# TobiasDeBruijn/UU-INFOGR-Raytracer

Hardware: AMD Instinct MI355X
Metric: Mray/s (primary+shadow+reflect) and fps at 1920×1080, 1/2/4/8 MI355X (higher is better)
Workload: dtype f32

## Files before the change

uu-infogr-raytracer_amd/csrc/rt_api.cpp:

```cpp
#include <hip/hip_runtime.h>

#include <algorithm>
#include <climits>
#include <cmath>
#include <cstdarg>
#include <cstdio>
#include <cstdlib>
#include <cstring>
#include <dlfcn.h>
#include <link.h>
#include <new>
#include <string>
#include <vector>

#include "../../include/raytracer_hip.h"
#include "rt_bands.h"
#include "rt_internal.h"
#include "rt_progressive.h"
#include "rt_scene.h"
#include "rt_view.h"

using namespace rtk;

namespace {
// ... 314 lines not shown

int view_params(rt_ctx* ctx, int W, int H, LaunchParams& lp, int ss = 0) {
    const int VH = ctx->view_height > 0 ? ctx->view_height << ss : H;
    if (H > VH)
        return fail(ctx, RT_ERR_INVALID_ARG, "frame height %d above the view height %d", H >> ss, ctx->view_height);
    if (ctx->view_ok && ctx->view_w == W && ctx->view_h == VH && ctx->view_rows == H &&
        std::memcmp(&ctx->view_cam, &ctx->cam, sizeof ctx->cam) == 0) {
        copy_view(ctx->view_lp, lp);
        return RT_OK;
    }
    int rc = view_fill(ctx, ctx->cam, W, VH, lp);
    if (rc != RT_OK) return rc;
    lp.row_order_n = row_order(lp, ctx->layout, lp.row_order);
    lp.H = H;
    copy_view(lp, ctx->view_lp);
    ctx->view_cam = ctx->cam, ctx->view_w = W, ctx->view_h = VH, ctx->view_rows = H, ctx->view_ok = true;
    return RT_OK;
}

void scene_params(const rt_ctx* ctx, const Device& d, LaunchParams& lp) {
    const SceneLayout& L = ctx->layout;
    const char* base = (const char*)d.d_scene;
    lp.sph = (const DevSphere*)(base + L.off_sph);
    lp.mat = (const DevMaterial*)(base + L.off_mat);
    lp.pl = (const DevPlane*)(base + L.off_pl);
    lp.li = (const DevLight*)(base + L.off_li);
    lp.scull = (const DevSphereCull*)(base + L.off_cull);
    lp.shcull = L.has_shcull ? (const DevShadowCull*)(base + L.off_shcull) : nullptr;
    lp.shg = L.has_shg ? (const DevShadowGrid*)(base + L.off_shg) : nullptr;
    lp.shgrid = L.has_shg ? (const unsigned long long*)(base + L.off_shgrid) : nullptr;
    lp.shslab = L.has_shg ? (const unsigned long long*)(base + L.off_shslab) : nullptr;
    lp.clus = L.n_clus ? (const DevCluster*)(base + L.off_clus) : nullptr;
    lp.shpre = L.has_shpre ? (const DevShadowCull*)(base + L.off_shpre) : nullptr;
    lp.n_clus = L.n_clus;
    lp.S = L.S, lp.P = L.P, lp.L = L.L, lp.limit = L.limit;
    lp.lights_a2_ok = L.lights_a2_ok ? 1 : 0;
    lp.uniform_plane = L.uniform_plane ? 1 : 0;
    lp.counters = ctx->counting ? d.d_counters : nullptr;
}

int view_tables(rt_ctx* ctx, Device& d, LaunchParams& lp, int ss = 0) {
    const int VH = ctx->view_height > 0 ? ctx->view_height << ss : lp.H;
    if (d.tab_w != lp.W || d.tab_h != VH || d.tab_pw != lp.pw || d.tab_ph != lp.ph || !d.d_view_tab) {
        std::vector<float> t((size_t)lp.W + (size_t)VH);
        view_table_values(lp.W, VH, lp.pw, lp.ph, t.data());
        HIP_TRY(ctx, hipDeviceSynchronize());
        int rc = grow(ctx, (void**)&d.d_view_tab, &d.view_tab_cap, t.size() * sizeof(float));
        if (rc != RT_OK) return rc;
        HIP_TRY(ctx, hipMemcpy(d.d_view_tab, t.data(), t.size() * sizeof(float), hipMemcpyHostToDevice));
        d.tab_w = lp.W, d.tab_h = VH, d.tab_pw = lp.pw, d.tab_ph = lp.ph;
    }
    lp.lxt = d.d_view_tab;
    lp.lyt = d.d_view_tab + lp.W;
    return RT_OK;
}

constexpr int ORDER_CANDIDATES = 4, ORDER_SAMPLES = 7;
constexpr float ORDER_MARGIN = 1.01f;
constexpr uint64_t ORDER_RETUNE = 1u << 14;

void order_collect(Device& d) {
    Device::OrderTuner& t = d.order;
    size_t keep = 0;
    for (size_t i = 0; i < t.pending.size(); ++i) {
        Device::OrderTuner::Probe& pr = t.pending[i];
        if (hipEventQuery(pr.b) != hipSuccess) {
// ... 538 lines not shown
        if (d.d_counters_diag) (void)hipFree(d.d_counters_diag);
        if (d.d_view_tab) (void)hipFree(d.d_view_tab);
        if (d.d_prog) (void)hipFree(d.d_prog);
        if (d.order.tiles.d_order) (void)hipFree(d.order.tiles.d_order);
        if (d.order.tiles.d_cost) (void)hipFree(d.order.tiles.d_cost);
        if (d.d_stage) (void)hipFree(d.d_stage);
        if (d.async_stream) (void)hipStreamDestroy(d.async_stream);
        if (d.stream) (void)hipStreamDestroy(d.stream);
    }
    delete ctx;
}

int rt_set_scene(rt_ctx* ctx, const rt_sphere* spheres, int n_spheres, const rt_plane* planes, int n_planes,
                 const rt_light* lights, int n_lights, rt_vec3 ambient, int recursion_limit) {
    if (!ctx) return fail(nullptr, RT_ERR_INVALID_ARG, "NULL context");
    if (n_spheres < 0 || n_planes < 0 || n_lights < 0 || (n_spheres && !spheres) || (n_planes && !planes) ||
        (n_lights && !lights))
        return fail(ctx, RT_ERR_INVALID_ARG, "rt_set_scene: bad primitive arrays");
    if (recursion_limit < 0) return fail(ctx, RT_ERR_INVALID_ARG, "recursion_limit must be >= 0");
    if (n_lights > RT_MAX_LIGHTS)
        return fail(ctx, RT_ERR_UNSUPPORTED, "n_lights %d > RT_MAX_LIGHTS (%d)", n_lights, RT_MAX_LIGHTS);
    if (recursion_limit > RT_MAX_RECURSION_LIMIT)
        return fail(ctx, RT_ERR_UNSUPPORTED, "recursion_limit %d > RT_MAX_RECURSION_LIMIT (%d)", recursion_limit,
                    RT_MAX_RECURSION_LIMIT);

    auto off = [](const char* name) {
        const char* v = std::getenv(name);
        return v && std::strcmp(v, "0") == 0;
    };
    SceneOptions opt;
    opt.shadow_grid = !off("RT_SHADOW_GRID");
    if (const char* cv = std::getenv("RT_TRACE_CLUSTERS")) opt.cluster_size = std::atoi(cv);
    opt.shadow_pre = !off("RT_SHADOW_PRE");
    opt.mirror_box = !off("RT_MIRROR_BOX");
    opt.dark_skip = !off("RT_DARK_SKIP");
    opt.prim_foot = !off("RT_PRIM_FOOT");
    opt.uniform_plane = !off("RT_UNIFORM_PLANE");
    SceneLayout L = scene_build(spheres, n_spheres, planes, n_planes, lights, n_lights, ambient, recursion_limit, opt);
    for (Device& d : ctx->dev) {
        DeviceGuard guard(d.id);
        HIP_TRY(ctx, hipDeviceSynchronize());
        int rc = grow(ctx, &d.d_scene, &d.scene_cap, L.bytes);
        if (rc != RT_OK) return rc;
        HIP_TRY(ctx, hipMemcpy(d.d_scene, L.host_blob.data(), L.bytes, hipMemcpyHostToDevice));
    }
    ctx->layout = std::move(L);
    ctx->has_scene = true;
    ctx->view_ok = false;
    ctx->scene_gen++;
    return RT_OK;
}

int rt_set_view_height(rt_ctx* ctx, int view_height) {
    if (!ctx || view_height < 0) return fail(ctx, RT_ERR_INVALID_ARG, "rt_set_view_height: bad arguments");
    ctx->view_height = view_height;
    return RT_OK;
}

int rt_set_supersampling(rt_ctx* ctx, int k) {
    if (!ctx) return fail(nullptr, RT_ERR_INVALID_ARG, "rt_set_supersampling: NULL context");
    if (k != 1 && k != 2 && k != 4 && k != 8)
        return fail(ctx, RT_ERR_INVALID_ARG, "rt_set_supersampling: factor %d is not 1, 2, 4 or 8", k);
    ctx->ss_log2 = k == 8 ? 3 : k == 4 ? 2 : k == 2 ? 1 : 0;
    return RT_OK;
}

// ... 991 lines not shown
```

uu-infogr-raytracer_amd/csrc/rt_internal.h:

```cpp
#pragma once
#include <stdint.h>

#include "rt_resolve.h"

namespace rtk {

struct DevSphere {
    float cx, cy, cz, r2;
};

enum : uint32_t { MAT_MIRROR = 1u, MAT_DIFFUSE = 2u, MAT_SPEC = 4u, MAT_DARK_OK = 8u };

enum : uint32_t { POW_GENERIC = 0u, POW_ONE = 1u, POW_HALF = 2u, POW_TWO = 3u };

struct DevMaterial {
    float kd[3];
    float amb[3];
    float ks[3];
    float n;
    float km[3];
    uint32_t flags;
    uint32_t pow_kind;
    uint32_t pad;
};
// ... 2 lines not shown
    float cx, cy, cz, cn;
    float nx, ny, nz, pad0;
    float e1x, e1y, e1z, pad1;
    float e2x, e2y, e2z, pad2;
};

struct DevLight {
    float px, py, pz, intensity;
    float a;
    float a2;
    float a4;
    float sh_t;
    float ax, ay, az, pad1;
    float ux, uy, uz, pad2;
    float vx, vy, vz, pad3;
};

struct DevSphereCull {
    float cx, cy, cz, rr;
};

struct DevCluster {
    float cx, cy, cz, R;
    unsigned long long members;
    unsigned long long pad;
};
constexpr int CLUSTER_SIZE = 8;
constexpr int MAX_CLUSTERS = 32;

struct DevShadowCull {
    float cu, cv, ca, rr;
};
constexpr long long SHADOW_CULL_MAX_ENTRIES = 1LL << 16;

constexpr int SHADOW_MERGE_L = 4;
constexpr int SHGRID_N = 64;
constexpr int SHGRID_SLABS = 32;
struct DevShadowGrid {
    float su, ou, sv, ov;
    float sa, oa;
    float bound;
    float far_k;
    float far_b;
    float bu0, bu1, bv0, bv1;
    float pad;
    unsigned long long always;
};

constexpr int COUNTER_SLOTS = 256;
constexpr int COUNTER_STRIDE = 8;
constexpr int COUNTER_WORDS = COUNTER_SLOTS * COUNTER_STRIDE;
enum : int { CNT_REFLECT = 1, CNT_SHADOW = 2, CNT_SHADOW_RUN = 3, CNT_SPHERE_RUN = 4, CNT_PLANE_RUN = 5 };
enum : int { CNT_EXTRA_PRIMARY = 0 };

struct PrimBox {
    int x0, x1, y0, y1;
};

struct PrimConst {
    float ocx, ocy, ocz, c;
};
constexpr int MAX_PRIM_CONST = 64;
struct PlaneFoot {
    float a, b, c;
};
constexpr int FOOT_MAX = 4;
// ... 48 lines not shown
    int n_frames;
    int32_t* out;
    unsigned long long out_frame_bytes;
    int out_fmt;
    unsigned char* enc_wire;
    uint32_t* enc_stage;
    int enc_tiles_x, enc_tpf, enc_frame0;
    unsigned long long* counters;
    CopyJob copy;
    int copy_z;
    int prim_const;
    PrimConst pc[MAX_PRIM_CONST];
    PrimBox pbox[MAX_PRIM_CONST];
    int row_order_n;
    int col_major;
    uint16_t row_order[ROW_ORDER_MAX];
    const uint32_t* tile_order;
    uint32_t* tile_cost;
    int ss_log2;
    int mbox_n;
    int mbox_plane[2];
    float mbox_tmax[2];
    PrimBox mbox[2][CULL_MIN_SPHERES];
    const DevView* views;
    int shutter_log2;
    int adapt_thr;
    int foot_n;
    PlaneFoot foot[FOOT_MAX];
    ResolveSum* prog_acc;
    int prog_first;
    int prog_n;
    int prog_pass[2];
    int uniform_plane;
};
constexpr int MIRROR_BOX_PLANES = 2;
constexpr int SINGLE_WPG = 4;
static_assert(sizeof(LaunchParams) < 4096, "LaunchParams is passed by value as the kernarg block (< 4 KiB)");

constexpr int OUT_TILES = 3;

constexpr int DIRECT_SMAX = 8;

enum : int { TV_DIRECT = 0, TV_BUNDLE = 1 };
enum : int { TM_PLAIN = 0, TM_STATS = 1, TM_TILES = 2, TM_SS = 3, TM_PATH = 4, TM_SHUTTER = 5, TM_ADAPT = 6, TM_PROG = 7 };
struct TraceVariant {
    int family;
    int gpow;
    int mode;
    int cls;
    int K;
    int wpg;
    int tord;
};

enum : unsigned { VF_GPOW = 1u, VF_STATS = 2u, VF_TILES = 4u, VF_SS = 8u, VF_PATH = 16u, VF_SHUTTER = 32u, VF_ADAPT = 64u, VF_PROG = 128u };
constexpr unsigned vf_cls(int c) { return (unsigned)c << 8; }
constexpr unsigned vf_wpg(int w) { return (unsigned)w << 12; }
constexpr unsigned vf_tord(int t) { return (unsigned)t << 16; }
constexpr int vf_cls_of(unsigned v) { return (int)(v >> 8 & 15u); }
constexpr int vf_wpg_of(unsigned v) { return (int)(v >> 12 & 15u); }
constexpr int vf_tord_of(unsigned v) { return (int)(v >> 16 & 3u); }
static_assert(DIRECT_SMAX < 16 && SINGLE_WPG < 16, "the variant word's 4-bit fields");
constexpr unsigned variant_word(const TraceVariant& v) {
    return (v.gpow ? VF_GPOW : 0u) | (v.mode == TM_STATS ? VF_STATS : 0u) | (v.mode == TM_TILES ? VF_TILES : 0u) |
           (v.mode == TM_SS ? VF_SS : 0u) | (v.mode == TM_PATH ? VF_PATH : 0u) |
           (v.mode == TM_SHUTTER ? VF_SHUTTER : 0u) | (v.mode == TM_ADAPT ? VF_ADAPT : 0u) | (v.mode == TM_PROG ? VF_PROG : 0u) |
// ... 83 lines not shown
```

uu-infogr-raytracer_amd/csrc/rt_kernel.hip:

```cpp
#include <hip/hip_runtime.h>

#include "rt_fastmath.h"
#include "rt_codec_common.h"
#include "rt_dark.h"
#include "rt_foot.h"
#include "rt_internal.h"
#include "rt_pow.h"
#include "rt_prims.h"
#include "rt_resolve.h"

constexpr int WG_THREADS = 64, TILE_W = 8, TILE_H = 8;

namespace rtk {

constexpr unsigned COPY_WAVES = 512;
__device__ __forceinline__ size_t band_dst(const CopyJob& j, unsigned i) {
    if (j.band_words == 0) return i;
    const unsigned k = i / j.band_words;
    return (size_t)k * j.dst_stride + (i - k * j.band_words);
}
__device__ __forceinline__ void copy_job(const CopyJob& j, size_t wg, size_t nwg) {
    const size_t lane = threadIdx.x & 63;
    const unsigned long long n = j.words, n4 = n / 4;
    const int4* __restrict__ s4 = (const int4*)j.src;
    const size_t step = nwg * 64;
    size_t i = wg * 64 + lane;
    if (j.band_words == 0) {
        int4* __restrict__ d4 = (int4*)j.dst;
        for (; i + 3 * step < n4; i += 4 * step) {
            const int4 a = s4[i], b = s4[i + step], c = s4[i + 2 * step], d = s4[i + 3 * step];
            d4[i] = a;
            d4[i + step] = b;
            d4[i + 2 * step] = c;
            d4[i + 3 * step] = d;
        }
        for (; i < n4; i += step) d4[i] = s4[i];
    } else {
        int4* __restrict__ d4 = (int4*)j.dst;
        const unsigned bq = j.band_words / 4, sq = (unsigned)(j.dst_stride / 4);
        for (unsigned c = (unsigned)i; c < (unsigned)n4; c += (unsigned)step) {
            const unsigned k = c / bq;
            d4[k * sq + (c - k * bq)] = s4[c];
// ... 297 lines not shown
        s += (RT_SHADOW_CAT && cat + 1 == sel_cat && (sel_lvl < 0 || lvl == sel_lvl)) ? n : 0u;
    }
    __device__ __forceinline__ void shadow_masks(int cat, unsigned long long m) {
        if (RT_SHADOW_CAT && cat + 1 == sel_cat && (sel_lvl < 0 || lvl == sel_lvl) && (threadIdx.x & 63) == 0)
            s += (unsigned)__builtin_popcountll(m);
    }
};

template <bool ST, int PATH = VIEW_ARGS, int SM>
__device__ __forceinline__ void add_counters(const LaunchParams& p, int lane, unsigned n_refl, unsigned n_shadow,
                                             const Tally<ST, SM>& tl) {
    if ((!PATH && blockIdx.z != (unsigned)p.copy_z) || p.counters == nullptr) return;
    const unsigned long long nf = !PATH && p.n_frames > 1 ? (unsigned long long)p.n_frames : 1ull;
    const unsigned b = wave_count(n_refl), c = wave_count(n_shadow);
    const unsigned slot = (blockIdx.y * gridDim.x + blockIdx.x) % COUNTER_SLOTS;
    unsigned long long* q = &p.counters[slot * COUNTER_STRIDE];
    if (lane == 0) {
        if (b) atomicAdd(q + CNT_REFLECT, b * nf);
        if (c) atomicAdd(q + CNT_SHADOW, c * nf);
    }
    if constexpr (ST) {
        const unsigned s = wave_count(tl.s), pl = wave_count(tl.pl), sh = wave_count(tl.sh);
        if (lane == 0) {
            if (sh) atomicAdd(q + CNT_SHADOW_RUN, sh * nf);
            if (s) atomicAdd(q + CNT_SPHERE_RUN, s * nf);
            if (pl) atomicAdd(q + CNT_PLANE_RUN, pl * nf);
        }
    }
}

#ifndef RT_UNIFORM_PLANE
#define RT_UNIFORM_PLANE 1
#endif

struct Hit {
    float t;
    int prim;
};
constexpr int HIT_NONE = 0x7fffffff;

__device__ __forceinline__ void take_primary(float t, int i, float& best, int& win) {
    const unsigned u = __float_as_uint(t) - 1u, ub = __float_as_uint(best) - 1u;
    win = u < ub ? i : win;
    best = __uint_as_float(min(u, ub) + 1u);
}
__device__ __forceinline__ void take_secondary(float t, int i, float& best, int& win) {
    const float tm = t - 0.01f;
    const bool b = __float_as_uint(tm) - 1u < __float_as_uint(best) - 1u;
    best = b ? t : best;
    win = b ? i : win;
}

__device__ __forceinline__ void plane_take(f3 o, f3 d, const DevPlane& q, int i, float& best, int& win) {
    const float num = ((-o.x * q.nx - o.y * q.ny) - o.z * q.nz) + q.cn;
    const float den = dot(d, mk(q.nx, q.ny, q.nz));
    const bool may = (num > 0.0f && den > 0.0f) || (num < 0.0f && den < 0.0f);
    if (__builtin_amdgcn_ballot_w64(may) != 0) take_primary(num / den, i, best, win);
}

__device__ __forceinline__ bool zero_or_nan(float v) { return !(v != 0.0f && v == v); }
__device__ __forceinline__ bool shadow_matters(f3 ph, float intensity, float att) {
    const float ia = intensity * att;
    const bool finite = __builtin_fabsf(ia) < __builtin_inff();
    return !(finite && zero_or_nan(ph.x) && zero_or_nan(ph.y) && zero_or_nan(ph.z));
}

template <typename T, typename F>
__device__ __forceinline__ void for_sphere_pairs(const LaunchParams& p, F body) {
    if constexpr (T::smax > 0) {
#pragma unroll
        for (int i = 0; i < T::smax; i += 2) {
            if (i >= p.S) break;
            body(i);
        }
    } else {
        for (int i = 0; i < p.S; i += 2) body(i);
    }
}

struct ShadowPreLane {
    float ou, ov, oa, ml;
};
__device__ __forceinline__ ShadowPreLane shadow_pre_lane(f3 hp, const DevLight& l) {
    ShadowPreLane q;
    q.ou = __builtin_fmaf(hp.z, l.uz, __builtin_fmaf(hp.y, l.uy, hp.x * l.ux));
    q.ov = __builtin_fmaf(hp.z, l.vz, __builtin_fmaf(hp.y, l.vy, hp.x * l.vx));
    q.oa = __builtin_fmaf(hp.z, l.az, __builtin_fmaf(hp.y, l.ay, hp.x * l.ax));
    const float l1 = __builtin_fabsf(q.ou) + __builtin_fabsf(q.ov) + __builtin_fabsf(q.oa);
    q.ml = l1 < 0x1p38f ? __builtin_fmaf(l1, 0x1.01p-8f, 0x1p-30f) : __builtin_inff();
    return q;
}
__device__ __forceinline__ bool shadow_pre_keep(const ShadowPreLane& q, const DevShadowCull& e) {
    const float wu = e.cu - q.ou, wv = e.cv - q.ov;
    const float T = e.rr + q.ml;
    const bool line = __builtin_fmaf(wu, wu, wv * wv) > T * T;
    const bool behind = q.oa - e.ca > q.ml;
    return !(line || behind);
}

template <bool A2OK, typename T>
__device__ __forceinline__ bool shadow_scan(const LaunchParams& p, f3 hp, const DevLight& l, int li, T& tl) {
    int blk = 0;
    if (A2OK && p.shpre != nullptr) {
        const ShadowPreLane q = shadow_pre_lane(hp, l);
        const DevShadowCull* e = p.shpre + (size_t)li * (size_t)(p.S + (p.S & 1));
        for_sphere_pairs<T>(p, [&](int i) {
            const DevShadowCull e0 = e[i], e1 = e[i + 1];
            const bool k0 = shadow_pre_keep(q, e0), k1 = shadow_pre_keep(q, e1);
            if (__builtin_amdgcn_ballot_w64(k0) != 0) {
                tl.shadow_sphere(blk == 0);
                blk = shadow_blocked<A2OK>(hp, l, false, p.sph[i]) ? 1 : blk;
            }
            if (__builtin_amdgcn_ballot_w64(k1) != 0) {
                tl.shadow_sphere(blk == 0);
                blk = shadow_blocked<A2OK>(hp, l, false, p.sph[i + 1]) ? 1 : blk;
            }
        });
        return blk != 0;
    }
    for_sphere_pairs<T>(p, [&](int i) {
        tl.shadow_sphere(blk == 0);
        const DevSphere s0 = p.sph[i], s1 = p.sph[i + 1];
        blk = shadow_blocked<A2OK>(hp, l, false, s0) ? 1 : blk;
        tl.shadow_sphere((blk == 0) & (i + 1 < p.S));
        blk = shadow_blocked<A2OK>(hp, l, false, s1) ? 1 : blk;
    });
    return blk != 0;
}

template <bool GPOW, typename T>
__device__ __forceinline__ f3 shade_direct(const LaunchParams& p, bool is_sphere, int prim, f3 hp, f3 d, float t, f3 sec,
                                           unsigned* n_shadow, T& tl) {
    const DevMaterial& m = p.mat[is_sphere ? prim : p.S + prim];
    const uint32_t flags = m.flags;
    f3 normal;
    float tile = 1.0f;
    bool dark = false;
    if (is_sphere) {
        const DevSphere& s = p.sph[prim];
        normal = normalize(sub(hp, mk(s.cx, s.cy, s.cz)));
    } else {
        const DevPlane& pl = p.pl[prim];
        normal = mk(pl.nx, pl.ny, pl.nz);
        const float u = dot(mk(pl.e1x, pl.e1y, pl.e1z), hp);
        const float v = dot(mk(pl.e2x, pl.e2y, pl.e2z), hp);
        tile = checker_tile(u, v);
        dark = (flags & MAT_DARK_OK) != 0 && dark_lane_ok(hp.x, hp.y, hp.z, t, dot(d, d), tile);
    }
    f3 col = mk(0.0f, 0.0f, 0.0f);
    if (flags & MAT_MIRROR) col = add(col, mul(sec, mk(m.km[0], m.km[1], m.km[2])));
    if ((flags & MAT_DIFFUSE) && !dark) {
        const f3 view = normalize(d);
        const float att = is_sphere ? sphere_att(t) : plane_att(t);
        const f3 kd = mk(m.kd[0], m.kd[1], m.kd[2]);
        const f3 ks = mk(m.ks[0], m.ks[1], m.ks[2]);
        const uint32_t pk = m.pow_kind;
        const float pn = m.n;
        for (int li = 0; li < p.L; ++li) {
            const DevLight& l = p.li[li];
            const bool l_ok = l.a2 > 0.0f && l.a2 < __builtin_inff();
            const f3 ldir = normalize(sub(mk(l.px, l.py, l.pz), hp));
            f3 ph = scale(kd, nmax0(dot(normal, ldir)));
            f3 spec = mk(0.0f, 0.0f, 0.0f);
            if (flags & MAT_SPEC) {
                const f3 rs = sub(ldir, scale(normal, 2.0f * dot(ldir, normal)));
                const float sp = spec_pow<GPOW>(nmax0(dot(view, normalize(rs))), pk, pn);
                spec = mul(ks, mk(sp, sp, sp));
            }
            ph = add(ph, spec);
            bool blocked = false;
            if (shadow_matters(ph, l.intensity, att)) {
                tl.shadow(true);
                blocked = l_ok ? shadow_scan<true>(p, hp, l, li, tl) : shadow_scan<false>(p, hp, l, li, tl);
            }
            const float inten = blocked ? 0.0f : l.intensity;
            const float ia = inten * att;
            f3 term = mul(mk(ia, ia, ia), ph);
            if (!is_sphere) {
                term = mul(term, mk(tile, tile, tile));
                term = mk(nmax0(term.x), nmax0(term.y), nmax0(term.z));
            }
            col = add(col, term);
        }
    }
    if (flags & MAT_DIFFUSE) *n_shadow += (unsigned)p.L << CNT_SHADOW_SHIFT;
    return add(col, mk(m.amb[0], m.amb[1], m.amb[2]));
}

template <typename T>
__device__ __forceinline__ f3 shade_plane_uniform(const LaunchParams& p, int plane, f3 hp, f3 d, float t, f3 sec,
                                                  unsigned* n_shadow, T& tl) {
    return shade_direct<false>(p, false, plane, hp, d, t, sec, n_shadow, tl);
}

__device__ __forceinline__ unsigned long long box_mask(const LaunchParams& p, const PrimBox* tab, int x, int y) {
    const int x_lo = __builtin_amdgcn_readlane(x, 0), x_hi = __builtin_amdgcn_readlane(x, 63);
    const int y_lo = __builtin_amdgcn_readlane(y, 0), y_hi = __builtin_amdgcn_readlane(y, 63);
    const int lane = threadIdx.x & 63;
    const bool in = lane < p.S;
    const PrimBox b = tab[in ? lane : 0];
    const bool cand = in & (b.x0 <= x_hi) & (b.x1 >= x_lo) & (b.y0 <= y_hi) & (b.y1 >= y_lo);
    return __builtin_amdgcn_ballot_w64(cand);
}
template <int PATH = VIEW_ARGS>
__device__ __forceinline__ unsigned long long prim_box_mask(const LaunchParams& p, int x, int y, int rec = 0) {
    return box_mask(p, ViewOf<PATH>{p, rec}.pbox(), x, y);
}
template <int PATH = VIEW_ARGS>
__device__ __forceinline__ unsigned mirror_box_masks(const LaunchParams& p, int x, int y, int rec = 0) {
    const ViewOf<PATH> vw{p, rec};
    unsigned m = 0;
    if (vw.mbox_n() > 0) {
        m = (unsigned)box_mask(p, vw.mbox(0), x, y);
        if (vw.mbox_n() > 1) m |= (unsigned)box_mask(p, vw.mbox(1), x, y) << 16;
    }
    return m;
}
template <int PATH = VIEW_ARGS>
__device__ __forceinline__ unsigned mirror_box_select(const LaunchParams& p, unsigned masks, float t, int prim, int rec = 0) {
    const ViewOf<PATH> vw{p, rec};
    const int pi = ~prim;
    const bool on0 = prim < 0 && pi == vw.mbox_plane(0) && t <= vw.mbox_tmax(0);
    const bool on1 = prim < 0 && pi == vw.mbox_plane(1) && t <= vw.mbox_tmax(1);
    if (__builtin_amdgcn_ballot_w64(!(on0 || on1)) != 0) return ~0u;
    unsigned m = 0;
// ... 1237 lines not shown
```

uu-infogr-raytracer_amd/csrc/rt_scene.h:

```cpp
#pragma once
#include <algorithm>
#include <cmath>
#include <cstdint>
#include <cstring>
#include <utility>
#include <vector>

#include "../../include/raytracer_hip.h"
#include "rt_dark.h"
#include "rt_internal.h"

namespace rtk {

struct H3 {
    float x, y, z;
};
inline H3 h3(rt_vec3 v) { return H3{v.x, v.y, v.z}; }
inline float hdot(H3 a, H3 b) { return ((a.x * b.x) + (a.y * b.y)) + (a.z * b.z); }
inline H3 hcross(H3 l, H3 r) {
    return H3{(l.y * r.z) - (l.z * r.y), (l.z * r.x) - (l.x * r.z), (l.x * r.y) - (l.y * r.x)};
}
inline H3 hnormalize(H3 a) {
    float s = 1.0f / std::sqrt(hdot(a, a));
    return H3{a.x * s, a.y * s, a.z * s};
// ... 3 lines not shown
inline DevMaterial dev_material(const rt_material& m, rt_vec3 ambient) {
    DevMaterial d;
    std::memset(&d, 0, sizeof d);
    d.kd[0] = m.kd.x, d.kd[1] = m.kd.y, d.kd[2] = m.kd.z;
    d.amb[0] = ambient.x * m.ka.x, d.amb[1] = ambient.y * m.ka.y, d.amb[2] = ambient.z * m.ka.z;
    d.ks[0] = m.ks.x, d.ks[1] = m.ks.y, d.ks[2] = m.ks.z;
    d.n = m.n;
    d.km[0] = m.km.x, d.km[1] = m.km.y, d.km[2] = m.km.z;
    d.flags = (hzero(m.km) ? 0u : MAT_MIRROR) | (hzero(m.kd) ? 0u : MAT_DIFFUSE) |
              ((!hzero(m.ks) && m.n > 0.0f) ? MAT_SPEC : 0u);
    d.pow_kind = m.n == 1.0f ? POW_ONE : m.n == 0.5f ? POW_HALF : m.n == 2.0f ? POW_TWO : POW_GENERIC;
    return d;
}

inline float shadow_threshold(float a2) {
    const float e = 0.001f;
    int ex = 0;
    (void)std::frexp(e, &ex);
    const double m = (double)e + std::ldexp(1.0, ex - 25);
    uint32_t eb;
    std::memcpy(&eb, &e, sizeof eb);
    const bool odd = (eb & 1u) != 0;
    const double T = m * (double)a2;
    float t = (float)T;
    if ((double)t < T || (!odd && (double)t == T)) t = std::nextafter(t, INFINITY);
    return t;
}

struct SceneLayout {
    int S = 0, P = 0, L = 0, limit = 0;
    size_t off_sph = 0, off_mat = 0, off_pl = 0, off_li = 0, off_cull = 0, off_shcull = 0, bytes = 0;
    size_t off_shg = 0, off_shgrid = 0, off_shslab = 0, off_clus = 0, off_shpre = 0;
    bool has_shpre = false;
    bool mirror_box = true;
    bool prim_foot = true;
    bool uniform_plane = true;
    int n_clus = 0;
    bool has_shcull = false;
    bool has_shg = false;
    std::vector<unsigned char> host_blob;
    bool generic_pow = false;
    bool lights_a2_ok = true;
    std::vector<DevSphere> host_sph;
    std::vector<DevPlane> host_pl;
};

struct SceneOptions {
    bool shadow_grid = true;
    bool shadow_pre = true;
    bool mirror_box = true;
    bool dark_skip = true;
    bool prim_foot = true;
    bool uniform_plane = true;
    int cluster_size = CLUSTER_SIZE;
};

struct Frame3 {
    double U[3], V[3], A[3];
};

inline double cell_lo(int k, float s, float o) { return ((double)k - 0x1p-22 * (std::fabs((double)k) + 2.0) - (double)o) / (double)s; }
inline double cell_hi(int k, float s, float o) {
    return ((double)(k + 1) + 0x1p-22 * (std::fabs((double)k + 1.0) + 2.0) - (double)o) / (double)s;
}
inline float down(double v) { float f = (float)v; return (double)f > v ? std::nextafter(f, -INFINITY) : f; }
inline float up(double v) { float f = (float)v; return (double)f < v ? std::nextafter(f, INFINITY) : f; }

inline void build_shadow_pre(const DevLight* li, int n_lights, const DevSphereCull* cull, int n_spheres, int s_pad,
                      DevShadowCull* out) {
    for (int j = 0; j < n_lights; ++j) {
        const DevLight& d = li[j];
        const bool l_ok = d.a >= 0x1p-40f && d.a <= 0x1p40f && d.a2 > 0.0f && d.a2 < INFINITY;
        for (int i = 0; i < s_pad; ++i) {
            DevShadowCull& e = out[(size_t)j * (size_t)s_pad + (size_t)i];
            if (i >= n_spheres) {
                e = DevShadowCull{INFINITY, 0.0f, 0.0f, 0.0f};
                continue;
            }
            const double c[3] = {cull[i].cx, cull[i].cy, cull[i].cz};
            const double clen = std::sqrt(c[0] * c[0] + c[1] * c[1] + c[2] * c[2]);
            const double cu = c[0] * d.ux + c[1] * d.uy + c[2] * d.uz;
            const double cv = c[0] * d.vx + c[1] * d.vy + c[2] * d.vz;
            const double ca = c[0] * d.ax + c[1] * d.ay + c[2] * d.az;
            const double l1 = std::fabs((double)(float)cu) + std::fabs((double)(float)cv) + std::fabs((double)(float)ca);
            const double mc = 0x1p-8 * l1 * (1.0 + 0x1p-20);
            const bool ok = l_ok && cull[i].rr >= 0x1p-50f && l1 < 0x1p38 && std::isfinite(cull[i].rr) && std::isfinite(clen);
            if (!ok) {
                e = DevShadowCull{0.0f, 0.0f, INFINITY, INFINITY};
                continue;
            }
            e.cu = (float)cu;
            e.cv = (float)cv;
            e.ca = std::nextafter((float)((double)(float)ca + mc), INFINITY);
            e.rr = std::nextafter((float)((double)cull[i].rr + 0x1p-18 * clen + mc), INFINITY);
        }
    }
}

inline void build_shadow_cull(const DevLight* li, int n_lights, const DevSphereCull* cull, int n_spheres,
                              DevShadowCull* sc) {
    for (int j = 0; j < n_lights; ++j)
        for (int i = 0; i < n_spheres; ++i) {
            const DevLight& d = li[j];
            const double c[3] = {cull[i].cx, cull[i].cy, cull[i].cz};
            const double clen = std::sqrt(c[0] * c[0] + c[1] * c[1] + c[2] * c[2]);
            DevShadowCull& e = sc[(size_t)j * (size_t)n_spheres + (size_t)i];
            e.cu = (float)(c[0] * d.ux + c[1] * d.uy + c[2] * d.uz);
            e.cv = (float)(c[0] * d.vx + c[1] * d.vy + c[2] * d.vz);
            e.ca = (float)(c[0] * d.ax + c[1] * d.ay + c[2] * d.az);
            e.rr = std::nextafter((float)((double)cull[i].rr + 0x1p-18 * clen), INFINITY);
        }
}

inline int build_clusters(const DevSphereCull* cull, int S, int size, DevCluster* out) {
    std::vector<std::vector<int>> todo(1, std::vector<int>((size_t)S)), groups;
    for (int i = 0; i < S; ++i) todo[0][(size_t)i] = i;
    while (!todo.empty()) {
        std::vector<int> g = std::move(todo.back());
        todo.pop_back();
        if ((int)g.size() <= size) {
            groups.push_back(std::move(g));
            continue;
        }
        double lo[3] = {INFINITY, INFINITY, INFINITY}, hi[3] = {-INFINITY, -INFINITY, -INFINITY};
        for (int i : g) {
            const double c[3] = {cull[i].cx, cull[i].cy, cull[i].cz};
            for (int k = 0; k < 3; ++k) lo[k] = std::fmin(lo[k], c[k]), hi[k] = std::fmax(hi[k], c[k]);
        }
        int ax = 0;
        for (int k = 1; k < 3; ++k)
            if (hi[k] - lo[k] > hi[ax] - lo[ax]) ax = k;
// ... 125 lines not shown
            unsigned long long m = 0;
            for (int j = 0; j < S; ++j)
                if (ok[j] && ca[j] + mB[j] > a_lo) m |= 1ull << j;
            slab[k + 1] = m;
        }
        if (!sa_ok) g.sa = 0.0f, g.oa = 0.0f;
    }
}

inline SceneLayout scene_build(const rt_sphere* spheres, int n_spheres, const rt_plane* planes, int n_planes,
                               const rt_light* lights, int n_lights, rt_vec3 ambient, int recursion_limit,
                               const SceneOptions& opt = SceneOptions{}) {
    SceneLayout L;
    L.S = n_spheres, L.P = n_planes, L.L = n_lights, L.limit = recursion_limit;
    auto al = [](size_t v) { return (v + 255) & ~(size_t)255; };
    const int s_pad = n_spheres + (n_spheres & 1);
    L.off_sph = 0;
    L.off_mat = al(L.off_sph + sizeof(DevSphere) * (size_t)s_pad);
    L.off_pl = al(L.off_mat + sizeof(DevMaterial) * (size_t)(n_spheres + n_planes));
    L.off_li = al(L.off_pl + sizeof(DevPlane) * (size_t)n_planes);
    L.off_cull = al(L.off_li + sizeof(DevLight) * (size_t)n_lights);
    L.off_shcull = al(L.off_cull + sizeof(DevSphereCull) * (size_t)n_spheres);
    L.has_shcull = (long long)n_lights * (long long)n_spheres <= SHADOW_CULL_MAX_ENTRIES;
    L.has_shg = merged_class(n_spheres, n_lights, true) != 0 && opt.shadow_grid;
    L.off_shg = al(L.off_shcull + (L.has_shcull ? sizeof(DevShadowCull) * (size_t)n_lights * (size_t)n_spheres : 0));
    L.off_shgrid = al(L.off_shg + (L.has_shg ? sizeof(DevShadowGrid) * (size_t)n_lights : 0));
    L.off_shslab = al(L.off_shgrid + (L.has_shg ? sizeof(unsigned long long) * SHGRID_N * SHGRID_N * (size_t)n_lights : 0));
    L.off_clus = al(L.off_shslab + (L.has_shg ? sizeof(unsigned long long) * (SHGRID_SLABS + 2) * (size_t)n_lights : 0));
    const int csize = opt.cluster_size;
    const bool want_clus = n_spheres >= CULL_MIN_SPHERES && n_spheres <= 64 && csize >= 1;
    L.off_shpre = al(L.off_clus + (want_clus ? sizeof(DevCluster) * MAX_CLUSTERS : 0));
    L.has_shpre = n_spheres < CULL_MIN_SPHERES && n_lights >= 1 && opt.shadow_pre;
    L.mirror_box = opt.mirror_box;
    L.bytes = al(L.off_shpre + (L.has_shpre ? sizeof(DevShadowCull) * (size_t)n_lights * (size_t)s_pad : 0)) + 256;

    std::vector<unsigned char> blob(L.bytes, 0);
    DevSphere* sph = (DevSphere*)(blob.data() + L.off_sph);
    DevMaterial* mat = (DevMaterial*)(blob.data() + L.off_mat);
    DevPlane* pl = (DevPlane*)(blob.data() + L.off_pl);
    DevLight* li = (DevLight*)(blob.data() + L.off_li);
    DevSphereCull* cull = (DevSphereCull*)(blob.data() + L.off_cull);
    for (int i = 0; i < n_spheres; ++i) {
        const rt_sphere& s = spheres[i];
        sph[i] = DevSphere{s.center.x, s.center.y, s.center.z, s.radius * s.radius};
        mat[i] = dev_material(s.material, ambient);
        const double rr = std::sqrt((double)sph[i].r2) * (1.0 + 0x1p-8);
        cull[i] = DevSphereCull{sph[i].cx, sph[i].cy, sph[i].cz, std::nextafter((float)rr, INFINITY)};
    }
    for (int i = n_spheres; i < s_pad; ++i) sph[i] = DevSphere{NAN, NAN, NAN, NAN};
    L.host_sph.assign(sph, sph + n_spheres);
    for (int i = 0; i < n_planes; ++i) {
        const rt_plane& p = planes[i];
        const H3 n = h3(p.normal);
        DevPlane d;
        std::memset(&d, 0, sizeof d);
        d.cx = p.center.x, d.cy = p.center.y, d.cz = p.center.z;
        d.cn = hdot(h3(p.center), n);
        d.nx = n.x, d.ny = n.y, d.nz = n.z;
        H3 e1 = hnormalize(hcross(n, H3{1.0f, 0.0f, 0.0f}));
        if (e1.x == 0 && e1.y == 0 && e1.z == 0) e1 = hnormalize(hcross(n, H3{0.0f, 0.0f, 1.0f}));
        H3 e2 = hnormalize(hcross(n, e1));
        d.e1x = e1.x, d.e1y = e1.y, d.e1z = e1.z;
        d.e2x = e2.x, d.e2y = e2.y, d.e2z = e2.z;
        pl[i] = d;
        mat[n_spheres + i] = dev_material(p.material, ambient);
    }
    L.host_pl.assign(pl, pl + n_planes);
// ... 6 lines not shown
        d.px = p.x, d.py = p.y, d.pz = p.z, d.intensity = l.intensity;
        d.a = hdot(p, p);
        d.a2 = 2.0f * d.a;
        d.a4 = 4.0f * d.a;
        d.sh_t = shadow_threshold(d.a2);
        if (!(d.a2 > 0.0f && d.a2 < INFINITY)) L.lights_a2_ok = false;
        const double len = std::sqrt((double)p.x * p.x + (double)p.y * p.y + (double)p.z * p.z);
        double A[3] = {0.0, 0.0, 1.0};
        if (len > 0 && std::isfinite(len)) A[0] = p.x / len, A[1] = p.y / len, A[2] = p.z / len;
        const double h[3] = {std::fabs(A[0]) < 0.9 ? 1.0 : 0.0, std::fabs(A[0]) < 0.9 ? 0.0 : 1.0, 0.0};
        double U[3] = {A[1] * h[2] - A[2] * h[1], A[2] * h[0] - A[0] * h[2], A[0] * h[1] - A[1] * h[0]};
        const double ul = std::sqrt(U[0] * U[0] + U[1] * U[1] + U[2] * U[2]);
        for (double& c : U) c /= ul;
        const double V[3] = {A[1] * U[2] - A[2] * U[1], A[2] * U[0] - A[0] * U[2], A[0] * U[1] - A[1] * U[0]};
        d.ax = (float)A[0], d.ay = (float)A[1], d.az = (float)A[2];
        d.ux = (float)U[0], d.uy = (float)U[1], d.uz = (float)U[2];
        d.vx = (float)V[0], d.vy = (float)V[1], d.vz = (float)V[2];
        li[i] = d;
        for (int k = 0; k < 3; ++k) frames[(size_t)i].U[k] = U[k], frames[(size_t)i].V[k] = V[k], frames[(size_t)i].A[k] = A[k];
    }
    L.prim_foot = opt.prim_foot;
    L.uniform_plane = opt.uniform_plane;
    if (opt.dark_skip)
        for (int i = 0; i < n_planes; ++i)
            if (plane_dark_ok(pl[i], mat[n_spheres + i], li, n_lights)) mat[n_spheres + i].flags |= MAT_DARK_OK;
    if (L.has_shg)
        for (int j = 0; j < n_lights; ++j)
            build_shadow_grid(li[j], frames[(size_t)j], sph, cull, n_spheres, ((DevShadowGrid*)(blob.data() + L.off_shg))[j],
                              (unsigned long long*)(blob.data() + L.off_shgrid) + (size_t)j * SHGRID_N * SHGRID_N,
                              (unsigned long long*)(blob.data() + L.off_shslab) + (size_t)j * (SHGRID_SLABS + 2));
    if (want_clus) L.n_clus = build_clusters(cull, n_spheres, csize, (DevCluster*)(blob.data() + L.off_clus));
    if (L.has_shcull) build_shadow_cull(li, n_lights, cull, n_spheres, (DevShadowCull*)(blob.data() + L.off_shcull));
    if (L.has_shpre) build_shadow_pre(li, n_lights, cull, n_spheres, s_pad, (DevShadowCull*)(blob.data() + L.off_shpre));
    for (int i = 0; i < n_spheres + n_planes; ++i)
        if ((mat[i].flags & MAT_SPEC) && mat[i].pow_kind == POW_GENERIC) L.generic_pow = true;
    L.host_blob = std::move(blob);
    return L;
}

}
```

Baseline: 304,600.

## Add per-light shadow group bounding discs for wave-level early-out of plane shadow rays

Builds a host-side hierarchy per light: spheres are greedily clustered into up to three groups, each enclosed by a conservative disc in the light's projected frame, plus a union disc over all groups. In the uniform-plane shading path, a wave-wide ballot against the union disc lets all lanes skip the per-sphere shadow-prefilter loop when no lane can be occluded. This is meant to remove the cost of scanning the sphere list for shadow rays that clearly miss everything. It adds scene-build work and a ballot plus an extra test per shadow ray. The group masks are computed but not yet used in the kernel.

```diff
diff --git a/uu-infogr-raytracer_amd/csrc/rt_api.cpp b/uu-infogr-raytracer_amd/csrc/rt_api.cpp
--- a/uu-infogr-raytracer_amd/csrc/rt_api.cpp
+++ b/uu-infogr-raytracer_amd/csrc/rt_api.cpp
@@ -370,6 +370,7 @@
     lp.shslab = L.has_shg ? (const unsigned long long*)(base + L.off_shslab) : nullptr;
     lp.clus = L.n_clus ? (const DevCluster*)(base + L.off_clus) : nullptr;
     lp.shpre = L.has_shpre ? (const DevShadowCull*)(base + L.off_shpre) : nullptr;
+    lp.shgrp = L.has_shgrp ? (const DevShadowGroups*)(base + L.off_shgrp) : nullptr;
     lp.n_clus = L.n_clus;
     lp.S = L.S, lp.P = L.P, lp.L = L.L, lp.limit = L.limit;
     lp.lights_a2_ok = L.lights_a2_ok ? 1 : 0;
@@ -974,6 +975,7 @@
     opt.shadow_grid = !off("RT_SHADOW_GRID");
     if (const char* cv = std::getenv("RT_TRACE_CLUSTERS")) opt.cluster_size = std::atoi(cv);
     opt.shadow_pre = !off("RT_SHADOW_PRE");
+    opt.shadow_groups = !off("RT_SHADOW_GROUPS");
     opt.mirror_box = !off("RT_MIRROR_BOX");
     opt.dark_skip = !off("RT_DARK_SKIP");
     opt.prim_foot = !off("RT_PRIM_FOOT");
diff --git a/uu-infogr-raytracer_amd/csrc/rt_internal.h b/uu-infogr-raytracer_amd/csrc/rt_internal.h
--- a/uu-infogr-raytracer_amd/csrc/rt_internal.h
+++ b/uu-infogr-raytracer_amd/csrc/rt_internal.h
@@ -58,6 +58,14 @@
     float cu, cv, ca, rr;
 };
 constexpr long long SHADOW_CULL_MAX_ENTRIES = 1LL << 16;
+constexpr int SHADOW_GROUPS = 3;
+struct DevShadowGroups {
+    DevShadowCull uni;
+    DevShadowCull grp[SHADOW_GROUPS];
+    uint32_t mask[SHADOW_GROUPS];
+    uint32_t pad;
+};
+static_assert(sizeof(DevShadowGroups) % 16 == 0, "DevShadowGroups records are 16-byte aligned in the scene image");
 
 constexpr int SHADOW_MERGE_L = 4;
 constexpr int SHGRID_N = 64;
@@ -172,6 +180,7 @@
     int prog_n;
     int prog_pass[2];
     int uniform_plane;
+    const DevShadowGroups* shgrp;
 };
 constexpr int MIRROR_BOX_PLANES = 2;
 constexpr int SINGLE_WPG = 4;
diff --git a/uu-infogr-raytracer_amd/csrc/rt_kernel.hip b/uu-infogr-raytracer_amd/csrc/rt_kernel.hip
--- a/uu-infogr-raytracer_amd/csrc/rt_kernel.hip
+++ b/uu-infogr-raytracer_amd/csrc/rt_kernel.hip
@@ -8,6 +8,7 @@
 #include "rt_pow.h"
 #include "rt_prims.h"
 #include "rt_resolve.h"
+#include "rt_shadow_pre.h"
 
 constexpr int WG_THREADS = 64, TILE_W = 8, TILE_H = 8;
 
@@ -371,6 +372,9 @@
 #ifndef RT_UNIFORM_PLANE
 #define RT_UNIFORM_PLANE 1
 #endif
+#ifndef RT_SHADOW_GROUPS
+#define RT_SHADOW_GROUPS 1
+#endif
 
 struct Hit {
     float t;
@@ -417,31 +421,16 @@
     }
 }
 
-struct ShadowPreLane {
-    float ou, ov, oa, ml;
-};
-__device__ __forceinline__ ShadowPreLane shadow_pre_lane(f3 hp, const DevLight& l) {
-    ShadowPreLane q;
-    q.ou = __builtin_fmaf(hp.z, l.uz, __builtin_fmaf(hp.y, l.uy, hp.x * l.ux));
-    q.ov = __builtin_fmaf(hp.z, l.vz, __builtin_fmaf(hp.y, l.vy, hp.x * l.vx));
-    q.oa = __builtin_fmaf(hp.z, l.az, __builtin_fmaf(hp.y, l.ay, hp.x * l.ax));
-    const float l1 = __builtin_fabsf(q.ou) + __builtin_fabsf(q.ov) + __builtin_fabsf(q.oa);
-    q.ml = l1 < 0x1p38f ? __builtin_fmaf(l1, 0x1.01p-8f, 0x1p-30f) : __builtin_inff();
-    return q;
-}
-__device__ __forceinline__ bool shadow_pre_keep(const ShadowPreLane& q, const DevShadowCull& e) {
-    const float wu = e.cu - q.ou, wv = e.cv - q.ov;
-    const float T = e.rr + q.ml;
-    const bool line = __builtin_fmaf(wu, wu, wv * wv) > T * T;
-    const bool behind = q.oa - e.ca > q.ml;
-    return !(line || behind);
-}
-
-template <bool A2OK, typename T>
+template <bool A2OK, bool GROUPS, typename T>
 __device__ __forceinline__ bool shadow_scan(const LaunchParams& p, f3 hp, const DevLight& l, int li, T& tl) {
     int blk = 0;
     if (A2OK && p.shpre != nullptr) {
-        const ShadowPreLane q = shadow_pre_lane(hp, l);
+        const ShadowPreLane q = shadow_pre_lane(hp.x, hp.y, hp.z, l);
+        if constexpr (GROUPS) {
+            if (p.shgrp != nullptr &&
+                __builtin_amdgcn_ballot_w64(shadow_pre_keep(shadow_pre_widen(q, SHADOW_UNION_WIDEN), p.shgrp[li].uni)) == 0)
+                return false;
+        }
         const DevShadowCull* e = p.shpre + (size_t)li * (size_t)(p.S + (p.S & 1));
         for_sphere_pairs<T>(p, [&](int i) {
             const DevShadowCull e0 = e[i], e1 = e[i + 1];
@@ -467,7 +456,7 @@
     return blk != 0;
 }
 
-template <bool GPOW, typename T>
+template <bool GPOW, bool GROUPS = false, typename T>
 __device__ __forceinline__ f3 shade_direct(const LaunchParams& p, bool is_sphere, int prim, f3 hp, f3 d, float t, f3 sec,
                                            unsigned* n_shadow, T& tl) {
     const DevMaterial& m = p.mat[is_sphere ? prim : p.S + prim];
@@ -510,7 +499,7 @@
             bool blocked = false;
             if (shadow_matters(ph, l.intensity, att)) {
                 tl.shadow(true);
-                blocked = l_ok ? shadow_scan<true>(p, hp, l, li, tl) : shadow_scan<false>(p, hp, l, li, tl);
+                blocked = l_ok ? shadow_scan<true, GROUPS>(p, hp, l, li, tl) : shadow_scan<false, false>(p, hp, l, li, tl);
             }
             const float inten = blocked ? 0.0f : l.intensity;
             const float ia = inten * att;
@@ -529,7 +518,7 @@
 template <typename T>
 __device__ __forceinline__ f3 shade_plane_uniform(const LaunchParams& p, int plane, f3 hp, f3 d, float t, f3 sec,
                                                   unsigned* n_shadow, T& tl) {
-    return shade_direct<false>(p, false, plane, hp, d, t, sec, n_shadow, tl);
+    return shade_direct<false, RT_SHADOW_GROUPS != 0>(p, false, plane, hp, d, t, sec, n_shadow, tl);
 }
 
 __device__ __forceinline__ unsigned long long box_mask(const LaunchParams& p, const PrimBox* tab, int x, int y) {
diff --git a/uu-infogr-raytracer_amd/csrc/rt_scene.h b/uu-infogr-raytracer_amd/csrc/rt_scene.h
--- a/uu-infogr-raytracer_amd/csrc/rt_scene.h
+++ b/uu-infogr-raytracer_amd/csrc/rt_scene.h
@@ -59,6 +59,8 @@
     size_t off_sph = 0, off_mat = 0, off_pl = 0, off_li = 0, off_cull = 0, off_shcull = 0, bytes = 0;
     size_t off_shg = 0, off_shgrid = 0, off_shslab = 0, off_clus = 0, off_shpre = 0;
     bool has_shpre = false;
+    size_t off_shgrp = 0;
+    bool has_shgrp = false;
     bool mirror_box = true;
     bool prim_foot = true;
     bool uniform_plane = true;
@@ -75,6 +77,7 @@
 struct SceneOptions {
     bool shadow_grid = true;
     bool shadow_pre = true;
+    bool shadow_groups = true;
     bool mirror_box = true;
     bool dark_skip = true;
     bool prim_foot = true;
@@ -124,6 +127,118 @@
     }
 }
 
+inline void enclosing_disc(const double* x, const double* y, const double* r, const std::vector<int>& idx, double* cx, double* cy) {
+    auto far = [&](double px, double py) {
+        double f = 0.0;
+        for (int i : idx) f = std::max(f, std::hypot(x[i] - px, y[i] - py) + r[i]);
+        return f;
+    };
+    double bx = x[idx[0]], by = y[idx[0]], br = r[idx[0]];
+    double x0 = bx, x1 = bx, y0 = by, y1 = by;
+    for (int i : idx) {
+        if (r[i] > br) bx = x[i], by = y[i], br = r[i];
+        x0 = std::min(x0, x[i]), x1 = std::max(x1, x[i]), y0 = std::min(y0, y[i]), y1 = std::max(y1, y[i]);
+    }
+    for (int i : idx)
+        for (int j : idx) {
+            const double d = std::hypot(x[j] - x[i], y[j] - y[i]);
+            const double span = 0.5 * (d + r[i] + r[j]);
+            if (j <= i || !(d > 0.0) || span <= br || span <= r[i] || span <= r[j]) continue;
+            const double t = (span - r[i]) / d;
+            bx = x[i] + (x[j] - x[i]) * t, by = y[i] + (y[j] - y[i]) * t, br = span;
+        }
+    *cx = bx, *cy = by;
+    if (far(bx, by) <= br * (1.0 + 0x1p-40)) return;
+    auto best_y = [&](double px, double* py) {
+        double lo = y0, hi = y1;
+        for (int k = 0; k < 52; ++k) {
+            const double a = lo + (hi - lo) / 3.0, b = hi - (hi - lo) / 3.0;
+            if (far(px, a) <= far(px, b)) hi = b; else lo = a;
+        }
+        *py = 0.5 * (lo + hi);
+        return far(px, *py);
+    };
+    double lo = x0, hi = x1, py = by;
+    for (int k = 0; k < 52; ++k) {
+        const double a = lo + (hi - lo) / 3.0, b = hi - (hi - lo) / 3.0;
+        if (best_y(a, &py) <= best_y(b, &py)) hi = b; else lo = a;
+    }
+    const double px = 0.5 * (lo + hi);
+    if (best_y(px, &py) < far(bx, by)) *cx = px, *cy = py;
+}
+
+inline DevShadowCull shadow_enclose(const DevShadowCull* m, int n) {
+    if (n == 0) return DevShadowCull{INFINITY, 0.0f, 0.0f, 0.0f};
+    std::vector<double> x((size_t)n), y((size_t)n), r((size_t)n);
+    std::vector<int> idx((size_t)n);
+    float ca = -INFINITY;
+    for (int i = 0; i < n; ++i) {
+        if (!(std::isfinite(m[i].rr) && std::isfinite(m[i].ca) && std::isfinite(m[i].cu) && std::isfinite(m[i].cv)))
+            return DevShadowCull{0.0f, 0.0f, INFINITY, INFINITY};
+        x[(size_t)i] = m[i].cu, y[(size_t)i] = m[i].cv, r[(size_t)i] = m[i].rr, idx[(size_t)i] = i;
+        ca = std::max(ca, m[i].ca);
+    }
+    double cx = 0.0, cy = 0.0;
+    enclosing_disc(x.data(), y.data(), r.data(), idx, &cx, &cy);
+    DevShadowCull e;
+    e.cu = (float)cx, e.cv = (float)cy, e.ca = ca;
+    double rr = 0.0;
+    for (int i = 0; i < n; ++i) rr = std::max(rr, std::hypot(x[(size_t)i] - (double)e.cu, y[(size_t)i] - (double)e.cv) + r[(size_t)i]);
+    e.rr = std::nextafter(up(rr * (1.0 + 0x1p-16)), INFINITY);
+    return e;
+}
+
+inline void build_shadow_groups(const DevShadowCull* pre, int n_lights, int n_spheres, int s_pad, DevShadowGroups* out,
+                                int groups = SHADOW_GROUPS) {
+    groups = std::max(1, std::min(groups, SHADOW_GROUPS));
+    for (int j = 0; j < n_lights; ++j) {
+        const DevShadowCull* e = pre + (size_t)j * (size_t)s_pad;
+        DevShadowGroups& g = out[j];
+        std::memset(&g, 0, sizeof g);
+        std::vector<std::vector<int>> cl;
+        std::vector<int> bad;
+        for (int i = 0; i < n_spheres; ++i) {
+            if (std::isfinite(e[i].rr) && std::isfinite(e[i].ca)) cl.push_back(std::vector<int>(1, i));
+            else bad.push_back(i);
+        }
+        const size_t room = (size_t)groups - (bad.empty() ? 0 : 1);
+        auto span = [&](const std::vector<int>& a, const std::vector<int>& b) {
+            double s = 0.0;
+            for (int p : a)
+                for (int q : b)
+                    s = std::max(s, 0.5 * (std::hypot((double)e[p].cu - (double)e[q].cu, (double)e[p].cv - (double)e[q].cv) +
+                                           (double)e[p].rr + (double)e[q].rr));
+            return s;
+        };
+        while (cl.size() > std::max<size_t>(room, 1)) {
+            size_t ba = 0, bb = 1;
+            double bs = INFINITY;
+            for (size_t a = 0; a < cl.size(); ++a)
+                for (size_t b = a + 1; b < cl.size(); ++b) {
+                    const double s = span(cl[a], cl[b]);
+                    if (s < bs) bs = s, ba = a, bb = b;
+                }
+            cl[ba].insert(cl[ba].end(), cl[bb].begin(), cl[bb].end());
+            cl.erase(cl.begin() + (std::ptrdiff_t)bb);
+        }
+        if (!bad.empty()) {
+            if (room == 0 && !cl.empty()) {
+                bad.insert(bad.end(), cl[0].begin(), cl[0].end());
+                cl.clear();
+            }
+            cl.insert(cl.begin(), bad);
+        }
+        for (int k = 0; k < SHADOW_GROUPS; ++k) {
+            std::vector<DevShadowCull> m;
+            if ((size_t)k < cl.size())
+                for (int i : cl[(size_t)k]) m.push_back(e[i]), g.mask[k] |= 1u << i;
+            g.grp[k] = shadow_enclose(m.data(), (int)m.size());
+        }
+        const int used = (int)std::min<size_t>(cl.size(), SHADOW_GROUPS);
+        g.uni = shadow_enclose(g.grp, used);
+    }
+}
+
 inline void build_shadow_cull(const DevLight* li, int n_lights, const DevSphereCull* cull, int n_spheres,
                               DevShadowCull* sc) {
     for (int j = 0; j < n_lights; ++j)
@@ -315,7 +430,9 @@
     L.off_shpre = al(L.off_clus + (want_clus ? sizeof(DevCluster) * MAX_CLUSTERS : 0));
     L.has_shpre = n_spheres < CULL_MIN_SPHERES && n_lights >= 1 && opt.shadow_pre;
     L.mirror_box = opt.mirror_box;
-    L.bytes = al(L.off_shpre + (L.has_shpre ? sizeof(DevShadowCull) * (size_t)n_lights * (size_t)s_pad : 0)) + 256;
+    L.off_shgrp = al(L.off_shpre + (L.has_shpre ? sizeof(DevShadowCull) * (size_t)n_lights * (size_t)s_pad : 0));
+    L.has_shgrp = L.has_shpre && opt.shadow_groups;
+    L.bytes = al(L.off_shgrp + (L.has_shgrp ? sizeof(DevShadowGroups) * (size_t)n_lights : 0)) + 256;
 
     std::vector<unsigned char> blob(L.bytes, 0);
     DevSphere* sph = (DevSphere*)(blob.data() + L.off_sph);
@@ -388,6 +505,9 @@
     if (want_clus) L.n_clus = build_clusters(cull, n_spheres, csize, (DevCluster*)(blob.data() + L.off_clus));
     if (L.has_shcull) build_shadow_cull(li, n_lights, cull, n_spheres, (DevShadowCull*)(blob.data() + L.off_shcull));
     if (L.has_shpre) build_shadow_pre(li, n_lights, cull, n_spheres, s_pad, (DevShadowCull*)(blob.data() + L.off_shpre));
+    if (L.has_shgrp)
+        build_shadow_groups((const DevShadowCull*)(blob.data() + L.off_shpre), n_lights, n_spheres, s_pad,
+                            (DevShadowGroups*)(blob.data() + L.off_shgrp));
     for (int i = 0; i < n_spheres + n_planes; ++i)
         if ((mat[i].flags & MAT_SPEC) && mat[i].pow_kind == POW_GENERIC) L.generic_pow = true;
     L.host_blob = std::move(blob);
diff --git a/uu-infogr-raytracer_amd/csrc/rt_shadow_pre.h b/uu-infogr-raytracer_amd/csrc/rt_shadow_pre.h
--- /dev/null
+++ b/uu-infogr-raytracer_amd/csrc/rt_shadow_pre.h
@@ -0,0 +1,40 @@
+#pragma once
+#include "rt_internal.h"
+
+#if defined(__HIPCC__)
+#define RT_SHPRE_FN __host__ __device__ inline
+#else
+#define RT_SHPRE_FN inline
+#endif
+
+namespace rtk {
+
+struct ShadowPreLane {
+    float ou, ov, oa, ml;
+};
+RT_SHPRE_FN ShadowPreLane shadow_pre_lane(float hx, float hy, float hz, const DevLight& l) {
+    ShadowPreLane q;
+    q.ou = __builtin_fmaf(hz, l.uz, __builtin_fmaf(hy, l.uy, hx * l.ux));
+    q.ov = __builtin_fmaf(hz, l.vz, __builtin_fmaf(hy, l.vy, hx * l.vx));
+    q.oa = __builtin_fmaf(hz, l.az, __builtin_fmaf(hy, l.ay, hx * l.ax));
+    const float l1 = __builtin_fabsf(q.ou) + __builtin_fabsf(q.ov) + __builtin_fabsf(q.oa);
+    q.ml = l1 < 0x1p38f ? __builtin_fmaf(l1, 0x1.01p-8f, 0x1p-30f) : __builtin_inff();
+    return q;
+}
+RT_SHPRE_FN bool shadow_pre_keep(const ShadowPreLane& q, const DevShadowCull& e) {
+    const float wu = e.cu - q.ou, wv = e.cv - q.ov;
+    const float T = e.rr + q.ml;
+    const bool line = __builtin_fmaf(wu, wu, wv * wv) > T * T;
+    const bool behind = q.oa - e.ca > q.ml;
+    return !(line || behind);
+}
+
+constexpr float SHADOW_GROUP_WIDEN = 1.0f + 0x1p-10f;
+constexpr float SHADOW_UNION_WIDEN = 1.0f + 0x1p-9f;
+RT_SHPRE_FN ShadowPreLane shadow_pre_widen(const ShadowPreLane& q, float k) {
+    ShadowPreLane w = q;
+    w.ml = q.ml * k;
+    return w;
+}
+
+}
```

Result: faster. 310,300, median of 6 (+1.9%).
